# iclavera/learning_to_adapt

Measured on AMD Instinct MI355X. Metric: controller-steps/sec (n_cand=2000, H=30, ens=5), higher is better.
Workload: dtype f32

## Files before the change

learning_to_adapt_amd/csrc/l2a_api.hip:

```cpp

#define L2A_PACK_KERNELS 1
#include "l2a_host.h"
#include "l2a_kernels.h"
#include "l2a_valu.h"
#include "l2a_adapt.h"
#include "l2a_mfma_launch.h"
#include "l2a_micro_pack.h"
#include "l2a_micro_launch.h"

#include <chrono>
#include <cmath>
#include <cstdio>
#include <cstdlib>
#include <cstring>
#include <string>
#include <vector>

#include <immintrin.h>
#include <unistd.h>

namespace {

std::string g_init_error;

// ... 66 lines not shown
int allow_big_lds(const l2a_ctx* ctx, K kernel, int bytes) {
    L2A_HIP(ctx, hipFuncSetAttribute(reinterpret_cast<const void*>(kernel),
                                     hipFuncAttributeMaxDynamicSharedMemorySize, bytes));
    return L2A_OK;
}

int split_mode_for(const l2a_model* md, int e_loop) {
    const int policy = md->ctx->split_policy;
    if (policy == 0) return 0;
    if ((e_loop & 1) && md->n_hidden >= 2 && policy == 1) return 2;
    return (e_loop >= 2) ? 1 : 0;
}

int choose_nt(const l2a_model* md, int m, int n, int e_loop, int sa_bytes_nt2, int other_bytes_nt2) {
    const int cus = md->ctx->num_cu > 0 ? md->ctx->num_cu : 256;
    if (2 * sa_bytes_nt2 + other_bytes_nt2 > md->ctx->lds_per_block) return 1;
    if (md->TPW >= 8 || md->OT >= 4) return 1;
    static const int force_nt = [] { const char* e = std::getenv("L2A_FORCE_NT"); return (e && (e[0] == '1' || e[0] == '2')) ? e[0] - '0' : 0; }();
    if (force_nt) return force_nt;
    const long long wg1 = (long long)m * ceil_div(n, 16);
    const long long wg2 = (long long)m * ceil_div(n, 32);
    const long long t = wg1 % cus;
    double cost1 = (double)((wg1 + cus - 1) / cus);
    if (wg1 > cus && t != 0 && 2 * t <= cus && split_mode_for(md, e_loop) != 0) cost1 = (double)(wg1 / cus) + 0.8;
    const double cost2 = (double)((wg2 + cus - 1) / cus) * 1.9;
    return (cost2 < cost1) ? 2 : 1;
}

int sa_elems_for(const l2a_model* md, int nt) {
    const int ht = md->H / 16;
    const int a = nt * ht;
    const int b = L2A_NW * nt * md->OT;
    return (a > b ? a : b) * 64;
}

int launch_rollout(l2a_model* md, L2AKParams& p, void* stream_v) {
    l2a_ctx* ctx = md->ctx;
    l2a_device_guard guard(ctx->device);
    hipStream_t stream = reinterpret_cast<hipStream_t>(stream_v);
    const int sets_needed = ctx->dry ? 0 : (p.mode == L2A_MODE_PER_BLOCK) ? (p.m < md->n_sets ? p.m : md->n_sets) : md->n_sets;
    for (int e = 0; e < sets_needed; ++e) {
        if (!md->weights_set[e]) return fail(ctx, L2A_ESTATE, "weight set " + std::to_string(e) + " was never set");
        if (!md->norm_set[e]) return fail(ctx, L2A_ESTATE, "normalisation of set " + std::to_string(e) + " was never set");
    }
    if (p.mode == L2A_MODE_PER_BLOCK && p.m > md->n_sets)
        return fail(ctx, L2A_EINVAL, "per-block mode needs one weight set per env/block");
    p.c_lo = 0; p.c_hi = p.n; p.done_total = 0;

    int kind = ctx->kernel_kind;
    if (kind == L2A_KERNEL_AUTO) kind = md->mfma_ok ? L2A_KERNEL_MFMA : L2A_KERNEL_VALU;
    if (kind == L2A_KERNEL_MFMA && !md->mfma_ok)
        return fail(ctx, L2A_EINVAL, "model shape is not eligible for the MFMA kernel "
                                     "(needs equal hidden widths of 128/256/512, obs_dim<=64, act_dim<=16)");

    const int e_loop0 = (p.mode == L2A_MODE_MEAN) ? md->n_sets : 1;
    const int cus0 = ctx->num_cu > 0 ? ctx->num_cu : 256;
    const int cst_set = 32 * md->KG0 + 48 * md->OT + md->n_hidden * md->H;
    auto lds_plan = [&](int nt_, int nseq, int x_bytes, int* lb_out, int* cst_off_out) {
        const int sa = sa_elems_for(md, nt_);
        const int ps_bytes = L2A_NW * nt_ * md->OT * 64 * 16;
        const int cst_bytes_all = nseq * cst_set * 4;
        int lb_ = 1, part_bytes = 0;
        if (md->n_hidden == 2 && ctx->batch_sets != 1) {
            const int cap = ctx->batch_sets > 0 ? ctx->batch_sets : 4;
            for (int lb = (nseq < cap ? nseq : cap); lb >= 2; --lb) {
                const int pbytes = lb * ps_bytes;
                if (lb * sa * 16 + pbytes + cst_bytes_all + x_bytes <= ctx->lds_per_block) {
                    lb_ = lb;
                    part_bytes = pbytes;
                    break;
                }
            }
        }
        *lb_out = lb_;
        *cst_off_out = ((lb_ > 1 ? lb_ : 2) * sa * 16 + part_bytes) / 16;
        return *cst_off_out * 16 + cst_bytes_all + x_bytes;
    };
    int front_k = 0;
    if (kind == L2A_KERNEL_MFMA) {
        const long long tiles1 = (long long)p.m * ceil_div(p.n, 16);
        int lb2 = 1, off2 = 0;
        if (ctx->double_policy != 0 && md->TPW == 8 && md->OT <= 3 && tiles1 >= 2LL * cus0 &&
            lds_plan(2, e_loop0, 0, &lb2, &off2) <= ctx->lds_per_block) {
            const long long D = tiles1 / (2LL * cus0);
            const long long R = tiles1 - 2LL * cus0 * D;
            if (R == 0 || 2 * R > 3LL * cus0) front_k = ceil_div(p.n, 32);
            else front_k = (int)((cus0 * D) / p.m);
            if (32LL * front_k >= p.n) front_k = ceil_div(p.n, 32);
        }
    }
    const int n_front = (32LL * front_k >= p.n) ? (front_k ? p.n : 0) : 32 * front_k;
    const int n_rest = p.n - n_front;

    bool micro = false;
    int mc_W = 0, mc_hi = 0, mc_quads = 0, smem_m = 0;
    long long mc_span = 0;
    if (kind == L2A_KERNEL_MFMA && n_rest > 0 && md->micro_ok && ctx->micro_policy != 0) {
        const long long tiles16 = (long long)p.m * ceil_div(n_rest, 16);
        const int quads = ceil_div(n_rest, 4);
        int W = cus0 / p.m;
        if (W > quads) W = quads;
        const int hi = W > 0 ? ceil_div(quads, W) : 99;
        if (hi >= 1 && hi <= 3) W = ceil_div(quads, hi);
        const int smem_need = l2a_mlp_micro_smem(md->H, md->KG0, md->n_hidden, e_loop0);
        const long long span = (long long)((p.mode == L2A_MODE_PER_BLOCK ? p.m : e_loop0) - 1) * md->set_stride * 4 +
                               l2a_mlp_micro_floats(md->H, md->KG0, md->n_hidden) * 4;
// ... 161 lines not shown
        rc = L2A_OK;
        if (rc != L2A_OK) return rc;
    } else {
        p.tiles_per_env = ceil_div(p.n, L2A_VT);
        const int smem = (md->in_dim + 2 * md->hmax + 3 * md->obs_dim + md->act_dim + 1) * L2A_VT * 4;
        if (smem > ctx->lds_per_block)
            return fail(ctx, L2A_EINVAL, "LDS budget exceeded by the VALU kernel (" + std::to_string(smem) + " B)");
        if (ctx->dry) {
            const int g[12] = {0, 0, 0, -1, 0, p.m * p.tiles_per_env, smem, 1, 0, 0, 0, 0};
            std::memcpy(ctx->dry, g, sizeof(g));
            return L2A_OK;
        }
        int rc = allow_big_lds(ctx, l2a_rollout_valu_k, smem);
        if (rc != L2A_OK) return rc;
        const dim3 grid((unsigned)(p.m * p.tiles_per_env)), block(256);
        hipLaunchKernelGGL(l2a_rollout_valu_k, grid, block, smem, stream, p);
    }
    L2A_HIP(ctx, hipGetLastError());
    return L2A_OK;
}

void model_shape(l2a_model* md, int obs_dim, int act_dim, int n_hidden, const int* hidden, int hidden_act, int output_act,
                 int n_sets, int mode) {
    md->obs_dim = obs_dim; md->act_dim = act_dim; md->in_dim = obs_dim + act_dim;
    md->n_hidden = n_hidden;
    md->hmax = 0;
    for (int i = 0; i < n_hidden; ++i) {
        md->hidden[i] = hidden[i];
        if (hidden[i] > md->hmax) md->hmax = hidden[i];
    }
    md->hidden_act = hidden_act; md->output_act = output_act;
    md->n_sets = n_sets; md->mode = mode;
    md->KG0 = ceil_div(md->in_dim, 16);
    md->OT = ceil_div(obs_dim, 16);
    md->mfma_ok = mfma_eligible(obs_dim, act_dim, n_hidden, hidden);
    md->H = md->mfma_ok ? hidden[0] : 0;
    md->TPW = md->mfma_ok ? hidden[0] / (16 * L2A_NW) : 0;
    md->micro_ok = md->mfma_ok && (md->H == 256 || md->H == 512);
    md->m_o4 = (md->micro_ok && md->OT == 2 && md->KG0 == 2 && n_hidden > 1 && obs_dim - 16 <= 4) ? 1 : 0;
}

void fill_model_params(const l2a_model* md, L2AKParams& p) {
    std::memset(&p, 0, sizeof(p));
    p.wblk = md->wblk;
    p.set_stride = md->set_stride;
    for (int i = 0; i < L2A_MAX_LAYERS; ++i) {
        p.raw_w[i] = md->raw_w[i];
        p.raw_b[i] = md->raw_b[i];
        p.hidden[i] = md->hidden[i];
    }
    p.pk_w0 = md->pk_w0; p.pk_wmid = md->pk_wmid; p.pk_wmid_stride = md->pk_wmid_stride;
    p.pk_wout = md->pk_wout; p.pk_bout = md->pk_bout; p.nm_off = md->nm_off;
    p.pk_m = md->pk_m; p.m_o4 = md->m_o4;
    p.m_nrec = md->micro_ok ? l2a_mlp_micro_nrec(md->H, md->KG0, md->n_hidden) : 0;
    p.n_hidden = md->n_hidden;
    p.obs_dim = md->obs_dim; p.act_dim = md->act_dim; p.in_dim = md->in_dim;
    p.hidden_act = md->hidden_act; p.output_act = md->output_act;
    p.mode = md->mode; p.n_sets = md->n_sets;
    p.KG0 = md->KG0; p.OT = md->OT; p.hmax = md->hmax;
    p.hid_floor = (md->hidden_act == L2A_ACT_RELU) ? 0.0f : -INFINITY;
    p.out_floor = (md->output_act == L2A_ACT_RELU) ? 0.0f : -INFINITY;
}

}

extern "C" {

int l2a_init(int device, l2a_ctx** out) {
    if (!out) return fail(nullptr, L2A_EINVAL, "l2a_init: out is null");
    *out = nullptr;
    int count = 0;
    hipError_t e = hipGetDeviceCount(&count);
    if (e != hipSuccess || count <= 0)
        return fail(nullptr, L2A_ENODEV, std::string("no HIP device visible: ") +
                                             (e != hipSuccess ? hipGetErrorString(e) : "device count is 0"));
    if (device < 0 || device >= count)
        return fail(nullptr, L2A_EINVAL, "device index " + std::to_string(device) + " out of range");
    hipDeviceProp_t prop;
    e = hipGetDeviceProperties(&prop, device);
    if (e != hipSuccess) return fail(nullptr, L2A_EHIP, std::string("hipGetDeviceProperties: ") + hipGetErrorString(e));
    std::string arch(prop.gcnArchName);
    if (arch.rfind("gfx950", 0) != 0)
        return fail(nullptr, L2A_ENODEV, "libl2a_hip.so is built for gfx950 only; device reports " + arch);
    e = hipSetDevice(device);
    if (e != hipSuccess) return fail(nullptr, L2A_EHIP, std::string("hipSetDevice: ") + hipGetErrorString(e));
    l2a_ctx* ctx = new l2a_ctx();
    ctx->device = device;
    ctx->num_cu = prop.multiProcessorCount;
    ctx->lds_per_block = (int)prop.sharedMemPerBlock;
    if (ctx->lds_per_block < 160 * 1024) ctx->lds_per_block = 160 * 1024;
    ctx->clock_khz = prop.clockRate;
    ctx->arch = arch;
    ctx->name = prop.name;
    e = hipHostMalloc(reinterpret_cast<void**>(&ctx->status_host), sizeof(unsigned int), hipHostMallocMapped);
    if (e == hipSuccess) {
        *ctx->status_host = 0;
        e = hipHostGetDevicePointer(reinterpret_cast<void**>(&ctx->status_dev), ctx->status_host, 0);
    }
    if (e != hipSuccess) {
        std::string msg = std::string("allocating the launch status word: ") + hipGetErrorString(e);
        delete ctx;
        return fail(nullptr, L2A_EHIP, msg);
    }
    const char* sp = std::getenv("L2A_SPLIT");
    if (sp && sp[0] >= '0' && sp[0] <= '2') ctx->split_policy = sp[0] - '0';
    const char* xa = std::getenv("L2A_XCD_ALIGN");
// ... 820 lines not shown
```

learning_to_adapt_amd/csrc/l2a_kernels.h:

```cpp
#pragma once

#include <hip/hip_runtime.h>

#include "../../include/l2a.h"

#define L2A_MAX_LAYERS 9
#define L2A_OTMAX 4
#define L2A_KG0MAX 5

typedef float f32x4 __attribute__((ext_vector_type(4)));

#define L2A_SC1 16

struct L2AKParams {
    const float* wblk;
    long long set_stride;
    long long raw_w[L2A_MAX_LAYERS];
    long long raw_b[L2A_MAX_LAYERS];
    long long pk_w0;
    long long pk_wmid;
    long long pk_wmid_stride;
    long long pk_wout;
    long long pk_bout;
    long long nm_off;
    int hidden[L2A_MAX_LAYERS];
    int n_hidden;
    int obs_dim, act_dim, in_dim;
    int hidden_act, output_act;
    int mode, n_sets;
    int KG0, OT;
    int sa_elems;
    int cst_set;
    int lb;
    int cst_off;
    int n_cst;
    float hid_floor, out_floor;
    long long pk_m;
    int m_nrec, m_o4;
    long long m_bytes;
    int mc_w, mc_r, mc_hi;
    int hmax;
    const float* obs0;
    const float* actions;
    float* returns_out;
    unsigned long long* best_key;
    float* state_out;
    const float* ret_in;
    double disc0;
    int obs_per_row;
    int m, n, h;
    int tiles_per_env;
    int c_lo, c_hi;
    int done_total;
    int cand_offset;
    double discount;
    l2a_reward rw;
    int split;
    int pl_units, pl_f, pl_r, pl_w;
    int split_from;
    unsigned int xtag;
    unsigned long long* xbuf;
    unsigned int* status;
    unsigned int spin_limit;
    unsigned long long* dbg;
    unsigned int* done_ctr;
    unsigned long long* mail_keys;
    unsigned long long* mail_seq_ptr;
    unsigned long long mail_seq;
    unsigned long long* next_keys;
};

__host__ __device__ inline void l2a_pack_decode(long long idx, int KG, int* k, int* u) {
    const int ii = (int)(idx & 3);
    const int lane = (int)((idx >> 2) & 63);
    const long long rest = idx >> 8;
    const int g = (int)(rest % KG);
    const int c = (int)(rest / KG);
    *k = 16 * g + 4 * (lane >> 4) + ii;
    *u = 16 * c + (lane & 15);
}

__device__ __forceinline__ float l2a_max_nan(float x, float f) { return __builtin_elementwise_maximum(x, f); }

__device__ __forceinline__ float l2a_act1(float x, int kind) {
    switch (kind) {
        case L2A_ACT_RELU: return l2a_max_nan(x, 0.0f);
        case L2A_ACT_TANH: return tanhf(x);
        case L2A_ACT_SIGMOID: return 1.0f / (1.0f + expf(-x));
        case L2A_ACT_SWISH: return x / (1.0f + expf(-x));
// ... 56 lines not shown
```

learning_to_adapt_amd/csrc/l2a_mfma.h:

```cpp
#pragma once

#include <type_traits>

#include "l2a_kernels.h"

#ifndef L2A_XEARLY
#define L2A_XEARLY 1
#endif

#ifndef L2A_NW
#define L2A_NW 4
#endif

typedef unsigned int u32x4 __attribute__((ext_vector_type(4)));
__device__ __forceinline__ __amdgpu_buffer_rsrc_t l2a_rsrc(const void* base, long long bytes) {
    return __builtin_amdgcn_make_buffer_rsrc(const_cast<void*>(base), 0, (int)bytes, 0x00020000);
}
__device__ __forceinline__ f32x4 l2a_ldw(__amdgpu_buffer_rsrc_t rs, int voff, int soff) {
    return __builtin_bit_cast(f32x4, __builtin_amdgcn_raw_buffer_load_b128(rs, voff, soff, 0));
}

template <bool GACT>
__device__ __forceinline__ f32x4 l2a_actv(f32x4 v, int kind, float floor) {
    if (GACT) return l2a_act4(v, kind);
// ... 4 lines not shown

__device__ __forceinline__ float l2a_sum_xor16(float x) {
    const unsigned int u = __float_as_uint(x);
    const auto r = __builtin_amdgcn_permlane16_swap(u, u, false, false);
    return __uint_as_float(r[0]) + __uint_as_float(r[1]);
}
__device__ __forceinline__ float l2a_sum_xor32(float x) {
    const unsigned int u = __float_as_uint(x);
    const auto r = __builtin_amdgcn_permlane32_swap(u, u, false, false);
    return __uint_as_float(r[0]) + __uint_as_float(r[1]);
}

#define L2A_MFMA4(a, b, c) __builtin_amdgcn_mfma_f32_4x4x1f32((a), (b), (c), 0, 0, 0)

#define L2A_OPAQUE(v) asm volatile("" : "+v"(v))

#ifndef L2A_TIMELINE
#define L2A_TS(slot)
#else
#define L2A_TS(slot)                                                                        \
    if (p.dbg && pairid == 0 && e < 8 && grp < 2) {                                         \
        unsigned long long ts_;                                                             \
        asm volatile("s_memtime %0\n\ts_waitcnt lgkmcnt(0)" : "=s"(ts_) : : "memory");       \
        if (lane == 0) p.dbg[(((long long)(grp * p.h + t) * 8 + e) * 8 + wave) * 16 + (slot)] = ts_; \
    }
#endif

#define L2A_STAGE_MFMA(CA, CB)                                                             \
    _Pragma("unroll") for (int ii = 0; ii < 4; ++ii)                                       \
        _Pragma("unroll") for (int nt = 0; nt < NT; ++nt)                                  \
            _Pragma("unroll") for (int tt = TW - 1; tt >= 0; --tt)    \
                acc[nt][tt] = L2A_MFMA(CA[tt][ii], CB[nt][ii], acc[nt][tt]);

#define L2A_STAGE(CA, CB, FA, FB, SOFF, IMM, GF)                                           \
    {                                                                                      \
        _Pragma("unroll") for (int tt = 0; tt < TW; ++tt)                                  \
            FA[tt] = l2a_ldw(rs, voff[tt] + (IMM), (SOFF));                                \
        _Pragma("unroll") for (int nt = 0; nt < NT; ++nt)                                  \
            FB[nt] = hin[(nt * HT + (GF)) * 64 + lane];                                    \
        L2A_STAGE_MFMA(CA, CB)                                                             \
         \
        __builtin_amdgcn_sched_group_barrier(0x100, NT, 0);                                \
        _Pragma("unroll") for (int tt = 0; tt < TW; ++tt) {                                \
            __builtin_amdgcn_sched_group_barrier(0x008, 4 * NT, 0);                        \
            __builtin_amdgcn_sched_group_barrier(0x020, 1, 0);                             \
        }                                                                                  \
        __builtin_amdgcn_sched_barrier(0);                                                 \
    }

#define L2A_PFT_MAX 6
#define L2A_PFT(TW_, OT_) ((OT_) <= 2 ? ((TW_) < L2A_PFT_MAX ? (TW_) : L2A_PFT_MAX) : ((TW_) < 2 ? (TW_) : 2))

template <int NT, int TW, int TPW, int OT, bool LAST>
__device__ __forceinline__ void l2a_hidden_gemm(__amdgpu_buffer_rsrc_t rs, __amdgpu_buffer_rsrc_t rsn,
                                                const int (&voff)[TPW], const int (&voffn)[TPW], int twn,
                                                int tile0, const f32x4* hin,
                                                f32x4 (&aA)[TPW], f32x4 (&aB)[TPW],
                                                f32x4 (&pfO)[TPW][OT], f32x4 (&acc)[NT][TPW], int lane,
                                                const float* bias_lds, f32x4 (&bias)[TPW], const int (&olane)[OT]) {
    constexpr int HT = L2A_NW * TPW;
    static_assert(HT % 4 == 0, "the k-group pipeline is unrolled by 4");
    f32x4 aC[TW], aD[TW], bA[NT], bB[NT], bC[NT], bD[NT];
#pragma unroll
    for (int nt = 0; nt < NT; ++nt) {
        bA[nt] = hin[(nt * HT + 0) * 64 + lane];
        bB[nt] = hin[(nt * HT + 1) * 64 + lane];
#pragma unroll
        for (int tt = 0; tt < TW; ++tt) acc[nt][tt] = (f32x4){0.f, 0.f, 0.f, 0.f};
    }
#pragma unroll
    for (int nt = 0; nt < NT; ++nt) { L2A_OPAQUE(bA[nt]); L2A_OPAQUE(bB[nt]); }
    __builtin_amdgcn_sched_barrier(0);

#pragma unroll 1
    for (int g = 0; g < HT - 4; g += 4) {
        const int soff = (g + 2) * 1024;
        L2A_STAGE(aA, bA, aC, bC, soff, 0, g + 2)
        L2A_STAGE(aB, bB, aD, bD, soff, 1024, g + 3)
        L2A_STAGE(aC, bC, aA, bA, soff, 2048, g + 4)
        L2A_STAGE(aD, bD, aB, bB, soff, 3072, g + 5)
    }
    L2A_STAGE(aA, bA, aC, bC, (HT - 2) * 1024, 0, HT - 2)
    L2A_STAGE(aB, bB, aD, bD, (HT - 2) * 1024, 1024, HT - 1)
    {
        if (LAST) {
#pragma unroll
            for (int tt = 0; tt < L2A_PFT(TW, OT); ++tt)
#pragma unroll
                for (int c = 0; c < OT; ++c)
                    if (((tt * OT + c) & 1) == 0)
                        pfO[tt][c] = l2a_ldw(rsn, olane[c] + (tile0 + tt) * 1024, c * HT * 1024);
        } else {
#pragma unroll
            for (int tt = 0; tt < TPW; ++tt)
                if (tt < twn) aA[tt] = l2a_ldw(rsn, voffn[tt], 0);
        }
        L2A_STAGE_MFMA(aC, bC)
        __builtin_amdgcn_sched_barrier(0);
    }
    {
#pragma unroll
        for (int tt = 0; tt < TW; ++tt) bias[tt] = *reinterpret_cast<const f32x4*>(bias_lds + 16 * tt);
        if (LAST) {
#pragma unroll
            for (int tt = 0; tt < L2A_PFT(TW, OT); ++tt)
#pragma unroll
                for (int c = 0; c < OT; ++c)
                    if (((tt * OT + c) & 1) == 1)
                        pfO[tt][c] = l2a_ldw(rsn, olane[c] + (tile0 + tt) * 1024, c * HT * 1024);
        } else {
#pragma unroll
            for (int tt = 0; tt < TPW; ++tt)
                if (tt < twn) aB[tt] = l2a_ldw(rsn, voffn[tt] + 1024, 0);
        }
        L2A_STAGE_MFMA(aD, bD)
        __builtin_amdgcn_sched_barrier(0);
    }
}

template <int NT, int TW, int TPW, int OT, int NPF, bool O4, class PF>
__device__ __forceinline__ void l2a_out_phase(const f32x4 (&hreg)[NT][TPW], f32x4 (&pfO)[TPW][OT],
                                              __amdgpu_buffer_rsrc_t rs_out, int tile0, PF prefetch,
                                              f32x4* pbuf, int chunk0, int lane, const int (&olane)[OT]) {
    constexpr int HT = L2A_NW * TPW;
    constexpr int CS = TPW / 2;
    constexpr int NCH = TW / CS;
    f32x4 a[TW][OT];
#pragma unroll
    for (int tt = 0; tt < TW; ++tt)
#pragma unroll
        for (int c = 0; c < OT; ++c)
            a[tt][c] = (tt < L2A_PFT(TW, OT)) ? pfO[tt][c]
                                              : l2a_ldw(rs_out, olane[c] + (tile0 + tt) * 1024, c * HT * 1024);
    prefetch();
    f32x4 acc[NCH][NT][OT];
#pragma unroll
    for (int ch = 0; ch < NCH; ++ch)
#pragma unroll
        for (int nt = 0; nt < NT; ++nt)
#pragma unroll
            for (int c = 0; c < OT; ++c) acc[ch][nt][c] = (f32x4){0.f, 0.f, 0.f, 0.f};
#pragma unroll
    for (int t2 = 0; t2 < CS; ++t2)
#pragma unroll
        for (int ii = 0; ii < 4; ++ii)
#pragma unroll
            for (int ch = 0; ch < NCH; ++ch)
#pragma unroll
                for (int nt = 0; nt < NT; ++nt)
#pragma unroll
                    for (int c = 0; c < OT; ++c)
                        acc[ch][nt][c] = (O4 && c == OT - 1)
                            ? L2A_MFMA4(a[ch * CS + t2][c][ii], hreg[nt][ch * CS + t2][ii], acc[ch][nt][c])
                            : L2A_MFMA(a[ch * CS + t2][c][ii], hreg[nt][ch * CS + t2][ii], acc[ch][nt][c]);
    {
        constexpr int NLATE = (TW - L2A_PFT(TW, OT)) * OT;
        constexpr int NMFMA = TW * 4 * NT * OT;
#pragma unroll
        for (int i = 0; i < NLATE; ++i) {
            __builtin_amdgcn_sched_group_barrier(0x020, 1, 0);
            __builtin_amdgcn_sched_group_barrier(0x008, 2, 0);
        }
        constexpr int PER = (NMFMA - 2 * NLATE) / NPF > 0 ? (NMFMA - 2 * NLATE) / NPF : 1;
#pragma unroll
        for (int i = 0; i < NPF; ++i) {
            __builtin_amdgcn_sched_group_barrier(0x008, PER, 0);
            __builtin_amdgcn_sched_group_barrier(0x020, 1, 0);
        }
    }
#pragma unroll
    for (int nt = 0; nt < NT; ++nt)
#pragma unroll
        for (int c = 0; c < OT; ++c)
            pbuf[((chunk0 * NT + nt) * OT + c) * 64 + lane] = (NCH == 2) ? acc[0][nt][c] + acc[NCH - 1][nt][c] : acc[0][nt][c];
}

template <int NT, int TPW, int OT, int KG0, bool GACT, int K0L = 4, bool N1 = false, bool O4 = false, bool FAN = false, bool WHOLE = false>
__global__ void __launch_bounds__(64 * L2A_NW) l2a_rollout_mfma_k(const L2AKParams p) {
    static_assert(!(FAN && WHOLE), "an instance is general, member fan or whole-tiles-only");
    constexpr bool NOHALF = FAN || WHOLE;
    constexpr int HT = L2A_NW * TPW;
    constexpr int TH = TPW / 2;
    static_assert(TPW % 2 == 0, "half members split a wave's tiles in two");
    constexpr int CST_BOUT = 32 * KG0 + 32 * OT;
    constexpr int CST_BHID = CST_BOUT + 16 * OT;
    constexpr int PS = L2A_NW * NT * OT * 64;
// ... 132 lines not shown
        for (int nt = 0; nt < NT; ++nt)
#pragma unroll
            for (int s = 0; s < 2; ++s)
#pragma unroll
                for (int ii = 0; ii < 4; ++ii)
                    dst[nt][s][ii] = __builtin_bit_cast(float, __builtin_amdgcn_raw_buffer_load_b32(ars, aoff[nt][s][ii], 0, 0));
    };
    f32x4 av[NT][2];
    float asq[NT];
    auto take_actions = [&](int t_fetch) {
#pragma unroll
        for (int nt = 0; nt < NT; ++nt) {
            av[nt][0] = av_next[nt][0];
            av[nt][1] = av_next[nt][1];
            float s = 0.0f;
#pragma unroll
            for (int ii = 0; ii < 4; ++ii) {
                s = fmaf(av[nt][0][ii], av[nt][0][ii], s);
                s = fmaf(av[nt][1][ii], av[nt][1][ii], s);
            }
            asq[nt] = s;
        }
        load_actions((t_fetch < p.h) ? t_fetch : p.h - 1, av_next);
    };
    load_actions(0, av_next);
    take_actions(1);

    float ret[NT];
#pragma unroll
    for (int nt = 0; nt < NT; ++nt) ret[nt] = p.ret_in ? p.ret_in[(long long)env * p.n + (valid[nt] ? cand[nt] : p.c_hi - 1)] : 0.0f;

    f32x4* hcur = buf0;
    f32x4* hoth = buf1;
    const float e_count = (float)e_loop;
    const float e_inv = 1.0f / e_count;
    double disc_pow = p.disc0;
    unsigned int spin_left = p.spin_limit;
    const unsigned int xtag0 = p.xtag;
    const __amdgpu_buffer_rsrc_t xrs = l2a_rsrc(p.xbuf, FAN ? (long long)n_pairs * e_loop * 2 * (NT * OT * 2 * 64 * 16)
                                                        : split ? (long long)n_pairs * 8 * (NT * OT * 2 * 64 * 16) : 16);

    constexpr int KG0P = (FAN && KG0 <= 2) ? KG0 : 1;
    f32x4 pfL0[KG0P][TPW];
    f32x4 pfA[TPW], pfB[TPW];
    f32x4 pfO[TPW][OT];
    int voff[TPW], voffh[TPW], voff0[TPW];
    const int tile0h = grp * (HT / 2) + wave * TH;
#pragma unroll
    for (int tt = 0; tt < TPW; ++tt) {
        voff[tt] = lane * 16 + (c0 + tt) * HT * 1024;
        voffh[tt] = lane * 16 + (tile0h + (tt < TH ? tt : 0)) * HT * 1024;
        voff0[tt] = lane * 16 + (c0 + tt) * KG0 * 1024;
    }
    const long long w0_bytes = (long long)HT * KG0 * 1024, wm_bytes = (long long)HT * HT * 1024,
                    wo_bytes = (long long)OT * HT * 1024;
    {
        const __amdgpu_buffer_rsrc_t r0 = l2a_rsrc(set_base(seq(0)) + p.pk_w0, w0_bytes);
#pragma unroll
        for (int g = 0; g < KG0P; ++g)
#pragma unroll
            for (int tt = 0; tt < TPW; ++tt) pfL0[g][tt] = l2a_ldw(r0, voff0[tt] + g * 1024, 0);
    }

    for (int t = 0; t < p.h; ++t) {
        f32x4 dsum[NT][OT], dgrp[NT][OT], qsh[NT][OT];
#pragma unroll
        for (int nt = 0; nt < NT; ++nt)
#pragma unroll
            for (int c = 0; c < OT; ++c) {
                dsum[nt][c] = (f32x4){0.f, 0.f, 0.f, 0.f};
                dgrp[nt][c] = (f32x4){0.f, 0.f, 0.f, 0.f};
                qsh[nt][c] = (f32x4){0.f, 0.f, 0.f, 0.f};
            }

        const unsigned int xtag = xtag0 + (unsigned int)(t + 1);
        constexpr int XREG = NT * OT * 2 * 64 * 16;
        auto xbase = [&](int g, int region) { return (((lpair * 2 + g) * 2 + (t & 1)) * 2 + region) * XREG + lane * 16; };
        auto xput = [&](int region, const f32x4 (&v)[NT][OT]) {
#pragma unroll
            for (int nt = 0; nt < NT; ++nt)
#pragma unroll
                for (int c = 0; c < OT; ++c)
#pragma unroll
                    for (int hh = 0; hh < 2; ++hh) {
                        u32x4 g;
                        g.x = xtag; g.y = __float_as_uint(v[nt][c][2 * hh]);
                        g.z = xtag; g.w = __float_as_uint(v[nt][c][2 * hh + 1]);
                        __builtin_amdgcn_raw_buffer_store_b128(g, xrs, xbase(grp, region) + ((nt * OT + c) * 2 + hh) * 1024, 0, L2A_SC1);
                    }
        };
        auto xget = [&](int region, f32x4 (&v)[NT][OT]) {
            bool ok = true;
#pragma unroll
            for (int nt = 0; nt < NT; ++nt)
#pragma unroll
                for (int c = 0; c < OT; ++c)
#pragma unroll
                    for (int hh = 0; hh < 2; ++hh) {
                        const u32x4 g = __builtin_amdgcn_raw_buffer_load_b128(
                            xrs, xbase(grp ^ 1, region) + ((nt * OT + c) * 2 + hh) * 1024, 0, L2A_SC1);
                        v[nt][c][2 * hh] = __uint_as_float(g.y);
                        v[nt][c][2 * hh + 1] = __uint_as_float(g.w);
                        ok = ok && (g.x == xtag) && (g.z == xtag);
                    }
            return ok;
        };

        bool xearly = false;
        u32x4 sw[2][NT][OT][2];
        for (int b0 = 0; b0 < n_seq; b0 += LB) {
            const int nb = (n_seq - b0 < LB) ? n_seq - b0 : LB;
            f32x4 hreg[NT][TPW];

            auto layer0 = [&](int j, auto last_tag) {
                constexpr bool last_l0 = decltype(last_tag)::value;
                const int i = b0 + j;
                const int e = seq(i);
                const float* wb = set_base(e);
                const float* nr = nrm + i * NRM_SET;
                const __amdgpu_buffer_rsrc_t rs_out = l2a_rsrc(wb + p.pk_wout, wo_bytes);
                L2A_TS(0)
                const __amdgpu_buffer_rsrc_t r0 = l2a_rsrc(wb + p.pk_w0, w0_bytes);
                f32x4 a[KG0][TPW];
#pragma unroll
                for (int g = 0; g < KG0; ++g)
#pragma unroll
                    for (int tt = 0; tt < TPW; ++tt)
                        a[g][tt] = (g < KG0P) ? pfL0[g < KG0P ? g : 0][tt] : l2a_ldw(r0, voff0[tt] + g * 1024, 0);
                L2A_TS(8)
                constexpr bool XPRE = (KG0 <= 2);
                auto norm_in = [&](int g, const f32x4& mu, const f32x4& iv, f32x4 (&x)[NT]) {
#pragma unroll
                    for (int nt = 0; nt < NT; ++nt) {
                        f32x4 sv = (f32x4){0.f, 0.f, 0.f, 0.f};
                        if (g < OT) sv = st[nt][g < OT ? g : 0];
                        f32x4 aa = (f32x4){0.f, 0.f, 0.f, 0.f};
                        if (g == ga0) aa = av[nt][0];
                        if (g == ga0 + 1) aa = av[nt][1];
#pragma unroll
                        for (int ii = 0; ii < 4; ++ii) x[nt][ii] = ((sv[ii] + aa[ii]) - mu[ii]) * iv[ii];
                    }
                };
                f32x4 xin[XPRE ? KG0 : 1][NT];
                if (XPRE) {
                    f32x4 mu[KG0], iv[KG0];
#pragma unroll
                    for (int g = 0; g < KG0; ++g) {
                        mu[g] = *reinterpret_cast<const f32x4*>(nr + 16 * g + 4 * qq);
                        iv[g] = *reinterpret_cast<const f32x4*>(nr + 16 * KG0 + 16 * g + 4 * qq);
                    }
                    __builtin_amdgcn_sched_barrier(0);
#pragma unroll
                    for (int g = 0; g < KG0; ++g) norm_in(g, mu[g], iv[g], xin[XPRE ? g : 0]);
                }
                f32x4 bias0[TPW];
#pragma unroll
                for (int tt = 0; tt < TPW; ++tt)
                    bias0[tt] = *reinterpret_cast<const f32x4*>(nr + CST_BHID + 16 * (c0 + tt) + 4 * qq);
                f32x4 acc[NT][TPW];
                auto l0_mfma = [&](auto npf_tag) {
                    constexpr int NPF = decltype(npf_tag)::value;
#pragma unroll
                    for (int nt = 0; nt < NT; ++nt)
#pragma unroll
                        for (int tt = 0; tt < TPW; ++tt) acc[nt][tt] = (f32x4){0.f, 0.f, 0.f, 0.f};
#pragma unroll
                    for (int g = 0; g < KG0; ++g) {
                        f32x4 xg[NT];
                        if (XPRE) {
#pragma unroll
                            for (int nt = 0; nt < NT; ++nt) xg[nt] = xin[XPRE ? g : 0][nt];
                        } else {
                            const f32x4 mu = *reinterpret_cast<const f32x4*>(nr + 16 * g + 4 * qq);
                            const f32x4 iv = *reinterpret_cast<const f32x4*>(nr + 16 * KG0 + 16 * g + 4 * qq);
                            norm_in(g, mu, iv, xg);
                        }
#pragma unroll
                        for (int ii = 0; ii < 4; ++ii) {
                            if (g == KG0 - 1 && ii >= K0L) continue;
#pragma unroll
                            for (int nt = 0; nt < NT; ++nt)
#pragma unroll
                                for (int tt = 0; tt < TPW; ++tt)
                                    acc[nt][tt] = L2A_MFMA(a[g][tt][ii], xg[nt][ii], acc[nt][tt]);
                        }
                    }
                    constexpr int NM = ((KG0 - 1) * 4 + K0L) * NT * TPW;
                    constexpr int PER = NM / (NPF > 0 ? NPF : 1) > 0 ? NM / (NPF > 0 ? NPF : 1) : 1;
                    __builtin_amdgcn_sched_group_barrier(0x020, (KG0 - KG0P) * TPW, 0);
#pragma unroll
                    for (int k = 0; k < NPF; ++k) {
                        __builtin_amdgcn_sched_group_barrier(0x008, PER, 0);
                        __builtin_amdgcn_sched_group_barrier(0x020, 1, 0);
                    }
                };
                if (N1) {
#pragma unroll
                    for (int tt = 0; tt < L2A_PFT(TPW, OT); ++tt)
#pragma unroll
                        for (int c = 0; c < OT; ++c)
                            pfO[tt][c] = l2a_ldw(rs_out, olane[c] + (c0 + tt) * 1024, c * HT * 1024);
                    l0_mfma(std::integral_constant<int, L2A_PFT(TPW, OT) * OT>{});
                } else if (!last_l0) {
                    const __amdgpu_buffer_rsrc_t r0n = l2a_rsrc(set_base(seq(i + 1)) + p.pk_w0, w0_bytes);
#pragma unroll
                    for (int g = 0; g < KG0P; ++g)
#pragma unroll
                        for (int tt = 0; tt < TPW; ++tt) pfL0[g][tt] = l2a_ldw(r0n, voff0[tt] + g * 1024, 0);
                    l0_mfma(std::integral_constant<int, KG0P * TPW>{});
                } else {
                    const int e0 = seq(b0);
                    const __amdgpu_buffer_rsrc_t rs1 = l2a_rsrc(set_base(e0) + p.pk_wmid, wm_bytes);
                    const bool next_half = !NOHALF && (e0 == e_shared) && n_hidden == 2;
                    if (next_half) {
#pragma unroll
                        for (int tt = 0; tt < TH; ++tt) {
                            pfA[tt] = l2a_ldw(rs1, voffh[tt], 0);
                            pfB[tt] = l2a_ldw(rs1, voffh[tt] + 1024, 0);
                        }
                        l0_mfma(std::integral_constant<int, 2 * TH>{});
                    } else {
#pragma unroll
                        for (int tt = 0; tt < TPW; ++tt) {
                            pfA[tt] = l2a_ldw(rs1, voff[tt], 0);
                            pfB[tt] = l2a_ldw(rs1, voff[tt] + 1024, 0);
                        }
                        l0_mfma(std::integral_constant<int, 2 * TPW>{});
                    }
                }
                L2A_TS(9)
#pragma unroll
                for (int tt = 0; tt < TPW; ++tt) {
#pragma unroll
                    for (int nt = 0; nt < NT; ++nt)
                        hreg[nt][tt] = l2a_actv<GACT>(acc[nt][tt] + bias0[tt], p.hidden_act, p.hid_floor);
                }
                L2A_TS(10)
                if (!N1) {
                    f32x4* hdst = (LB > 1) ? buf0 + j * p.sa_elems : hcur;
#pragma unroll
                    for (int tt = 0; tt < TPW; ++tt)
#pragma unroll
                        for (int nt = 0; nt < NT; ++nt) hdst[(nt * HT + c0 + tt) * 64 + lane] = hreg[nt][tt];
                }
                L2A_TS(1)
            };

            auto member = [&](int j, auto last_tag) {
                constexpr bool last_set = decltype(last_tag)::value;
                const int i = b0 + j;
                const int e = seq(i);
                const bool is_half = !NOHALF && last_set && (e == e_shared);
                const float* wb = set_base(e);
                const float* nr = nrm + i * NRM_SET;
                const __amdgpu_buffer_rsrc_t rs_out = l2a_rsrc(wb + p.pk_wout, wo_bytes);
                f32x4* pb = (LB > 1) ? pbase + j * PS : hoth;
                L2A_TS(2)
                if (!N1) {
                    f32x4 acc[NT][TPW], bias[TPW];
                    for (int l = 1; last_set && l < n_hidden - 1; ++l) {
                        const float* wl = wb + p.pk_wmid + (long long)(l - 1) * p.pk_wmid_stride;
                        const bool next_half = is_half && (l == n_hidden - 2);
                        l2a_hidden_gemm<NT, TPW, TPW, OT, false>(l2a_rsrc(wl, wm_bytes), l2a_rsrc(wl + p.pk_wmid_stride, wm_bytes),
                                                                 voff, next_half ? voffh : voff, next_half ? TH : TPW, 0,
                                                                 hcur, pfA, pfB, pfO, acc, lane,
                                                                 nr + CST_BHID + l * (16 * HT) + 16 * c0 + 4 * qq, bias, olane);
#pragma unroll
                        for (int tt = 0; tt < TPW; ++tt) {
#pragma unroll
                            for (int nt = 0; nt < NT; ++nt)
                                hoth[(nt * HT + c0 + tt) * 64 + lane] = l2a_actv<GACT>(acc[nt][tt] + bias[tt], p.hidden_act, p.hid_floor);
                        }
                        __syncthreads();
                        f32x4* tmp = hcur; hcur = hoth; hoth = tmp;
                    }
                    if (LB == 1) pb = hoth;
                    L2A_TS(15)
                    const f32x4* hin = (LB > 1) ? buf0 + j * p.sa_elems : hcur;
                    const __amdgpu_buffer_rsrc_t rs_last =
                        l2a_rsrc(wb + p.pk_wmid + (long long)(n_hidden - 2) * p.pk_wmid_stride, wm_bytes);
                    const float* bl = nr + CST_BHID + (n_hidden - 1) * (16 * HT);
                    if (!is_half) {
                        l2a_hidden_gemm<NT, TPW, TPW, OT, true>(rs_last, rs_out, voff, voff, TPW, c0, hin, pfA, pfB, pfO,
                                                                acc, lane, bl + 16 * c0 + 4 * qq, bias, olane);
#pragma unroll
                        for (int tt = 0; tt < TPW; ++tt) {
#pragma unroll
                            for (int nt = 0; nt < NT; ++nt)
                                hreg[nt][tt] = l2a_actv<GACT>(acc[nt][tt] + bias[tt], p.hidden_act, p.hid_floor);
                        }
                    } else {
                        l2a_hidden_gemm<NT, TH, TPW, OT, true>(rs_last, rs_out, voffh, voffh, TH, tile0h, hin, pfA, pfB,
                                                               pfO, acc, lane, bl + 16 * tile0h + 4 * qq, bias, olane);
#pragma unroll
                        for (int tt = 0; tt < TH; ++tt) {
#pragma unroll
                            for (int nt = 0; nt < NT; ++nt)
                                hreg[nt][tt] = l2a_actv<GACT>(acc[nt][tt] + bias[tt], p.hidden_act, p.hid_floor);
                        }
                    }
                }
                L2A_TS(3)
                if (last_set) {
                    const __amdgpu_buffer_rsrc_t r0n = l2a_rsrc(set_base(seq((i + 1 < n_seq) ? i + 1 : 0)) + p.pk_w0, w0_bytes);
                    auto pf_l0 = [&]() {
#pragma unroll
                        for (int g = 0; g < KG0P; ++g)
#pragma unroll
                            for (int tt = 0; tt < TPW; ++tt) pfL0[g][tt] = l2a_ldw(r0n, voff0[tt] + g * 1024, 0);
                    };
                    if (is_half) l2a_out_phase<NT, TH, TPW, OT, KG0P * TPW, O4>(hreg, pfO, rs_out, tile0h, pf_l0, pb, wave, lane, olane);
                    else l2a_out_phase<NT, TPW, TPW, OT, KG0P * TPW, O4>(hreg, pfO, rs_out, c0, pf_l0, pb, wave, lane, olane);
                } else {
                    const int en = seq(i + 1);
                    const __amdgpu_buffer_rsrc_t rsn = l2a_rsrc(set_base(en) + p.pk_wmid, wm_bytes);
                    if (!NOHALF && en == e_shared) {
                        l2a_out_phase<NT, TPW, TPW, OT, 2 * TH, O4>(hreg, pfO, rs_out, c0, [&]() {
#pragma unroll
                            for (int tt = 0; tt < TH; ++tt) {
                                pfA[tt] = l2a_ldw(rsn, voffh[tt], 0);
                                pfB[tt] = l2a_ldw(rsn, voffh[tt] + 1024, 0);
                            }
                        }, pb, wave, lane, olane);
                    } else {
                        l2a_out_phase<NT, TPW, TPW, OT, 2 * TPW, O4>(hreg, pfO, rs_out, c0, [&]() {
#pragma unroll
                            for (int tt = 0; tt < TPW; ++tt) {
                                pfA[tt] = l2a_ldw(rsn, voff[tt], 0);
                                pfB[tt] = l2a_ldw(rsn, voff[tt] + 1024, 0);
                            }
                        }, pb, wave, lane, olane);
                    }
                }
                L2A_TS(4)
            };
            for (int j = 0; j + 1 < nb; ++j) layer0(j, std::false_type{});
            layer0(nb - 1, std::true_type{});
            if (!N1) __syncthreads();
            for (int j = 0; j + 1 < nb; ++j) member(j, std::false_type{});
            member(nb - 1, std::true_type{});

            __syncthreads();
            constexpr bool XE_OK = L2A_XEARLY && !NOHALF && NT == 1 && OT <= 2 && KG0 <= 2;
            const bool xe = XE_OK && split == 2 && nb >= 2 && b0 + nb == n_seq;
            for (int jj = 0; jj < nb; ++jj) {
                const int j = (xe && wave == 0) ? (jj == 0 ? nb - 1 : jj - 1) : jj;
                const int i = b0 + j;
                const int e = seq(i);
                const bool is_half = !NOHALF && (e == e_shared);
                const float* nr = nrm + i * NRM_SET;
                const f32x4* pb = (LB > 1) ? pbase + j * PS : hoth;
                L2A_TS(5)
                if (e == e_half && !split) {
#pragma unroll
                    for (int nt = 0; nt < NT; ++nt)
#pragma unroll
                        for (int c = 0; c < OT; ++c) {
                            dsum[nt][c] = dgrp[nt][c];
                            dgrp[nt][c] = (f32x4){0.f, 0.f, 0.f, 0.f};
                        }
                }
#pragma unroll
                for (int c = 0; c < OT; ++c) {
                    f32x4 part[L2A_NW][NT];
#pragma unroll
                    for (int ch = 0; ch < L2A_NW; ++ch)
#pragma unroll
                        for (int nt = 0; nt < NT; ++nt) part[ch][nt] = pb[((ch * NT + nt) * OT + c) * 64 + lane];
                    const f32x4 bias = *reinterpret_cast<const f32x4*>(nr + CST_BOUT + 16 * c + 4 * qq);
                    const f32x4 omu = *reinterpret_cast<const f32x4*>(nr + 32 * KG0 + 16 * c + 4 * qq);
                    const f32x4 osd = *reinterpret_cast<const f32x4*>(nr + 32 * KG0 + 16 * OT + 16 * c + 4 * qq);
                    __builtin_amdgcn_sched_barrier(0);
#pragma unroll
                    for (int nt = 0; nt < NT; ++nt) {
                        static_assert(L2A_NW == 4, "the canonical tree below is written out for four waves");
                        f32x4 s = (part[0][nt] + part[1][nt]) + (part[2][nt] + part[3][nt]);
                        if (is_half) {
                            qsh[nt][c] = s;
                        } else {
                            if (O4 && c == OT - 1) {
#pragma unroll
                                for (int ii = 0; ii < 4; ++ii) s[ii] = l2a_sum_xor32(l2a_sum_xor16(s[ii]));
// ... 338 lines not shown
```

Baseline: 702.6.

## Use one weight-block buffer resource with scalar offsets and peel first hidden-GEMM stage

Replaces the per-set, per-layer buffer resource descriptors with a single descriptor covering the whole weight block, addressing each set and layer through int scalar offsets. This removes repeated 128-bit descriptor construction and the SGPR pressure that comes with it. It also peels the first stage of the hidden GEMM when NT==1, so the accumulator is seeded by the first MFMA instead of being zeroed, and adds sched_group_barrier hints to interleave the loads. Models whose weights exceed 2 GiB are now rejected from the MFMA path.

```diff
diff --git a/learning_to_adapt_amd/csrc/l2a_api.hip b/learning_to_adapt_amd/csrc/l2a_api.hip
--- a/learning_to_adapt_amd/csrc/l2a_api.hip
+++ b/learning_to_adapt_amd/csrc/l2a_api.hip
@@ -142,6 +142,8 @@
     if (kind == L2A_KERNEL_MFMA && !md->mfma_ok)
         return fail(ctx, L2A_EINVAL, "model shape is not eligible for the MFMA kernel "
                                      "(needs equal hidden widths of 128/256/512, obs_dim<=64, act_dim<=16)");
+    if (kind == L2A_KERNEL_MFMA && md->set_stride * md->n_sets * 4 >= (1LL << 31))
+        return fail(ctx, L2A_EINVAL, "the model's weight block exceeds 2 GiB: not eligible for the MFMA kernel (use the VALU kernel)");
 
     const int e_loop0 = (p.mode == L2A_MODE_MEAN) ? md->n_sets : 1;
     const int cus0 = ctx->num_cu > 0 ? ctx->num_cu : 256;
@@ -409,6 +411,12 @@
     p.pk_w0 = md->pk_w0; p.pk_wmid = md->pk_wmid; p.pk_wmid_stride = md->pk_wmid_stride;
     p.pk_wout = md->pk_wout; p.pk_bout = md->pk_bout; p.nm_off = md->nm_off;
     p.pk_m = md->pk_m; p.m_o4 = md->m_o4;
+    if (md->mfma_ok && md->set_stride * md->n_sets * 4 < (1LL << 31)) {
+        p.wb_total = (int)(md->set_stride * md->n_sets * 4);
+        p.wb_set = (int)(md->set_stride * 4);
+        p.wb_w0 = (int)(md->pk_w0 * 4); p.wb_wmid = (int)(md->pk_wmid * 4);
+        p.wb_wmid_stride = (int)(md->pk_wmid_stride * 4); p.wb_wout = (int)(md->pk_wout * 4);
+    }
     p.m_nrec = md->micro_ok ? l2a_mlp_micro_nrec(md->H, md->KG0, md->n_hidden) : 0;
     p.n_hidden = md->n_hidden;
     p.obs_dim = md->obs_dim; p.act_dim = md->act_dim; p.in_dim = md->in_dim;
diff --git a/learning_to_adapt_amd/csrc/l2a_kernels.h b/learning_to_adapt_amd/csrc/l2a_kernels.h
--- a/learning_to_adapt_amd/csrc/l2a_kernels.h
+++ b/learning_to_adapt_amd/csrc/l2a_kernels.h
@@ -35,6 +35,7 @@
     int cst_off;
     int n_cst;
     float hid_floor, out_floor;
+    int wb_total, wb_set, wb_w0, wb_wmid, wb_wmid_stride, wb_wout;
     long long pk_m;
     int m_nrec, m_o4;
     long long m_bytes;
diff --git a/learning_to_adapt_amd/csrc/l2a_mfma.h b/learning_to_adapt_amd/csrc/l2a_mfma.h
--- a/learning_to_adapt_amd/csrc/l2a_mfma.h
+++ b/learning_to_adapt_amd/csrc/l2a_mfma.h
@@ -80,7 +80,7 @@
 #define L2A_PFT(TW_, OT_) ((OT_) <= 2 ? ((TW_) < L2A_PFT_MAX ? (TW_) : L2A_PFT_MAX) : ((TW_) < 2 ? (TW_) : 2))
 
 template <int NT, int TW, int TPW, int OT, bool LAST>
-__device__ __forceinline__ void l2a_hidden_gemm(__amdgpu_buffer_rsrc_t rs, __amdgpu_buffer_rsrc_t rsn,
+__device__ __forceinline__ void l2a_hidden_gemm(__amdgpu_buffer_rsrc_t rs, int sb, int sbn,
                                                 const int (&voff)[TPW], const int (&voffn)[TPW], int twn,
                                                 int tile0, const f32x4* hin,
                                                 f32x4 (&aA)[TPW], f32x4 (&aB)[TPW],
@@ -93,23 +93,57 @@
     for (int nt = 0; nt < NT; ++nt) {
         bA[nt] = hin[(nt * HT + 0) * 64 + lane];
         bB[nt] = hin[(nt * HT + 1) * 64 + lane];
-#pragma unroll
-        for (int tt = 0; tt < TW; ++tt) acc[nt][tt] = (f32x4){0.f, 0.f, 0.f, 0.f};
-    }
-#pragma unroll
-    for (int nt = 0; nt < NT; ++nt) { L2A_OPAQUE(bA[nt]); L2A_OPAQUE(bB[nt]); }
-    __builtin_amdgcn_sched_barrier(0);
-
+    }
+    constexpr bool PEEL = (NT == 1);
+    if constexpr (PEEL) {
+#pragma unroll
+        for (int tt = 0; tt < TW; ++tt) aC[tt] = l2a_ldw(rs, voff[tt], sb + 2 * 1024);
+#pragma unroll
+        for (int nt = 0; nt < NT; ++nt) bC[nt] = hin[(nt * HT + 2) * 64 + lane];
+#pragma unroll
+        for (int ii = 0; ii < 4; ++ii)
+#pragma unroll
+            for (int nt = 0; nt < NT; ++nt)
+#pragma unroll
+                for (int tt = TW - 1; tt >= 0; --tt)
+                    acc[nt][tt] = L2A_MFMA(aA[tt][ii], bA[nt][ii], (ii == 0 ? (f32x4){0.f, 0.f, 0.f, 0.f} : acc[nt][tt]));
+        __builtin_amdgcn_sched_group_barrier(0x100, NT, 0);
+#pragma unroll
+        for (int tt = 0; tt < TW; ++tt) {
+            __builtin_amdgcn_sched_group_barrier(0x008, 4 * NT, 0);
+            __builtin_amdgcn_sched_group_barrier(0x020, 1, 0);
+        }
+        __builtin_amdgcn_sched_barrier(0);
+#pragma unroll
+        for (int nt = 0; nt < NT; ++nt) { L2A_OPAQUE(bB[nt]); L2A_OPAQUE(bC[nt]); }
+        __builtin_amdgcn_sched_barrier(0);
 #pragma unroll 1
-    for (int g = 0; g < HT - 4; g += 4) {
-        const int soff = (g + 2) * 1024;
-        L2A_STAGE(aA, bA, aC, bC, soff, 0, g + 2)
-        L2A_STAGE(aB, bB, aD, bD, soff, 1024, g + 3)
-        L2A_STAGE(aC, bC, aA, bA, soff, 2048, g + 4)
-        L2A_STAGE(aD, bD, aB, bB, soff, 3072, g + 5)
-    }
-    L2A_STAGE(aA, bA, aC, bC, (HT - 2) * 1024, 0, HT - 2)
-    L2A_STAGE(aB, bB, aD, bD, (HT - 2) * 1024, 1024, HT - 1)
+        for (int g = 1; g < HT - 3; g += 4) {
+            const int soff = sb + (g + 2) * 1024;
+            L2A_STAGE(aB, bB, aD, bD, soff, 0, g + 2)
+            L2A_STAGE(aC, bC, aA, bA, soff, 1024, g + 3)
+            L2A_STAGE(aD, bD, aB, bB, soff, 2048, g + 4)
+            L2A_STAGE(aA, bA, aC, bC, soff, 3072, g + 5)
+        }
+    } else {
+#pragma unroll
+        for (int nt = 0; nt < NT; ++nt)
+#pragma unroll
+            for (int tt = 0; tt < TW; ++tt) acc[nt][tt] = (f32x4){0.f, 0.f, 0.f, 0.f};
+#pragma unroll
+        for (int nt = 0; nt < NT; ++nt) { L2A_OPAQUE(bA[nt]); L2A_OPAQUE(bB[nt]); }
+        __builtin_amdgcn_sched_barrier(0);
+#pragma unroll 1
+        for (int g = 0; g < HT - 4; g += 4) {
+            const int soff = sb + (g + 2) * 1024;
+            L2A_STAGE(aA, bA, aC, bC, soff, 0, g + 2)
+            L2A_STAGE(aB, bB, aD, bD, soff, 1024, g + 3)
+            L2A_STAGE(aC, bC, aA, bA, soff, 2048, g + 4)
+            L2A_STAGE(aD, bD, aB, bB, soff, 3072, g + 5)
+        }
+        L2A_STAGE(aA, bA, aC, bC, sb + (HT - 2) * 1024, 0, HT - 2)
+    }
+    L2A_STAGE(aB, bB, aD, bD, sb + (HT - 2) * 1024, 1024, HT - 1)
     {
         if (LAST) {
 #pragma unroll
@@ -117,11 +151,11 @@
 #pragma unroll
                 for (int c = 0; c < OT; ++c)
                     if (((tt * OT + c) & 1) == 0)
-                        pfO[tt][c] = l2a_ldw(rsn, olane[c] + (tile0 + tt) * 1024, c * HT * 1024);
+                        pfO[tt][c] = l2a_ldw(rs, olane[c] + (tile0 + tt) * 1024, sbn + c * HT * 1024);
         } else {
 #pragma unroll
             for (int tt = 0; tt < TPW; ++tt)
-                if (tt < twn) aA[tt] = l2a_ldw(rsn, voffn[tt], 0);
+                if (tt < twn) aA[tt] = l2a_ldw(rs, voffn[tt], sbn);
         }
         L2A_STAGE_MFMA(aC, bC)
         __builtin_amdgcn_sched_barrier(0);
@@ -135,11 +169,11 @@
 #pragma unroll
                 for (int c = 0; c < OT; ++c)
                     if (((tt * OT + c) & 1) == 1)
-                        pfO[tt][c] = l2a_ldw(rsn, olane[c] + (tile0 + tt) * 1024, c * HT * 1024);
+                        pfO[tt][c] = l2a_ldw(rs, olane[c] + (tile0 + tt) * 1024, sbn + c * HT * 1024);
         } else {
 #pragma unroll
             for (int tt = 0; tt < TPW; ++tt)
-                if (tt < twn) aB[tt] = l2a_ldw(rsn, voffn[tt] + 1024, 0);
+                if (tt < twn) aB[tt] = l2a_ldw(rs, voffn[tt] + 1024, sbn);
         }
         L2A_STAGE_MFMA(aD, bD)
         __builtin_amdgcn_sched_barrier(0);
@@ -148,7 +182,7 @@
 
 template <int NT, int TW, int TPW, int OT, int NPF, bool O4, class PF>
 __device__ __forceinline__ void l2a_out_phase(const f32x4 (&hreg)[NT][TPW], f32x4 (&pfO)[TPW][OT],
-                                              __amdgpu_buffer_rsrc_t rs_out, int tile0, PF prefetch,
+                                              __amdgpu_buffer_rsrc_t rs_out, int so_out, int tile0, PF prefetch,
                                               f32x4* pbuf, int chunk0, int lane, const int (&olane)[OT]) {
     constexpr int HT = L2A_NW * TPW;
     constexpr int CS = TPW / 2;
@@ -159,7 +193,7 @@
 #pragma unroll
         for (int c = 0; c < OT; ++c)
             a[tt][c] = (tt < L2A_PFT(TW, OT)) ? pfO[tt][c]
-                                              : l2a_ldw(rs_out, olane[c] + (tile0 + tt) * 1024, c * HT * 1024);
+                                              : l2a_ldw(rs_out, olane[c] + (tile0 + tt) * 1024, so_out + c * HT * 1024);
     prefetch();
     f32x4 acc[NCH][NT][OT];
 #pragma unroll
@@ -398,15 +432,13 @@
         voffh[tt] = lane * 16 + (tile0h + (tt < TH ? tt : 0)) * HT * 1024;
         voff0[tt] = lane * 16 + (c0 + tt) * KG0 * 1024;
     }
-    const long long w0_bytes = (long long)HT * KG0 * 1024, wm_bytes = (long long)HT * HT * 1024,
-                    wo_bytes = (long long)OT * HT * 1024;
-    {
-        const __amdgpu_buffer_rsrc_t r0 = l2a_rsrc(set_base(seq(0)) + p.pk_w0, w0_bytes);
-#pragma unroll
-        for (int g = 0; g < KG0P; ++g)
-#pragma unroll
-            for (int tt = 0; tt < TPW; ++tt) pfL0[g][tt] = l2a_ldw(r0, voff0[tt] + g * 1024, 0);
-    }
+    const __amdgpu_buffer_rsrc_t rW = l2a_rsrc(p.wblk, p.wb_total);
+    const int wb_set = p.wb_set;
+    auto set_off = [&](int i) { return (per_block ? env : seq(i)) * wb_set; };
+#pragma unroll
+    for (int g = 0; g < KG0P; ++g)
+#pragma unroll
+        for (int tt = 0; tt < TPW; ++tt) pfL0[g][tt] = l2a_ldw(rW, voff0[tt] + g * 1024, set_off(0) + p.wb_w0);
 
     for (int t = 0; t < p.h; ++t) {
         f32x4 dsum[NT][OT], dgrp[NT][OT], qsh[NT][OT];
@@ -462,17 +494,15 @@
                 constexpr bool last_l0 = decltype(last_tag)::value;
                 const int i = b0 + j;
                 const int e = seq(i);
-                const float* wb = set_base(e);
+                const int so = set_off(i);
                 const float* nr = nrm + i * NRM_SET;
-                const __amdgpu_buffer_rsrc_t rs_out = l2a_rsrc(wb + p.pk_wout, wo_bytes);
                 L2A_TS(0)
-                const __amdgpu_buffer_rsrc_t r0 = l2a_rsrc(wb + p.pk_w0, w0_bytes);
                 f32x4 a[KG0][TPW];
 #pragma unroll
                 for (int g = 0; g < KG0; ++g)
 #pragma unroll
                     for (int tt = 0; tt < TPW; ++tt)
-                        a[g][tt] = (g < KG0P) ? pfL0[g < KG0P ? g : 0][tt] : l2a_ldw(r0, voff0[tt] + g * 1024, 0);
+                        a[g][tt] = (g < KG0P) ? pfL0[g < KG0P ? g : 0][tt] : l2a_ldw(rW, voff0[tt] + g * 1024, so + p.wb_w0);
                 L2A_TS(8)
                 constexpr bool XPRE = (KG0 <= 2);
                 auto norm_in = [&](int g, const f32x4& mu, const f32x4& iv, f32x4 (&x)[NT]) {
@@ -545,31 +575,31 @@
                     for (int tt = 0; tt < L2A_PFT(TPW, OT); ++tt)
 #pragma unroll
                         for (int c = 0; c < OT; ++c)
-                            pfO[tt][c] = l2a_ldw(rs_out, olane[c] + (c0 + tt) * 1024, c * HT * 1024);
+                            pfO[tt][c] = l2a_ldw(rW, olane[c] + (c0 + tt) * 1024, so + p.wb_wout + c * HT * 1024);
                     l0_mfma(std::integral_constant<int, L2A_PFT(TPW, OT) * OT>{});
                 } else if (!last_l0) {
-                    const __amdgpu_buffer_rsrc_t r0n = l2a_rsrc(set_base(seq(i + 1)) + p.pk_w0, w0_bytes);
+                    const int son = set_off(i + 1) + p.wb_w0;
 #pragma unroll
                     for (int g = 0; g < KG0P; ++g)
 #pragma unroll
-                        for (int tt = 0; tt < TPW; ++tt) pfL0[g][tt] = l2a_ldw(r0n, voff0[tt] + g * 1024, 0);
+                        for (int tt = 0; tt < TPW; ++tt) pfL0[g][tt] = l2a_ldw(rW, voff0[tt] + g * 1024, son);
                     l0_mfma(std::integral_constant<int, KG0P * TPW>{});
                 } else {
                     const int e0 = seq(b0);
-                    const __amdgpu_buffer_rsrc_t rs1 = l2a_rsrc(set_base(e0) + p.pk_wmid, wm_bytes);
+                    const int so1 = set_off(b0) + p.wb_wmid;
                     const bool next_half = !NOHALF && (e0 == e_shared) && n_hidden == 2;
                     if (next_half) {
 #pragma unroll
                         for (int tt = 0; tt < TH; ++tt) {
-                            pfA[tt] = l2a_ldw(rs1, voffh[tt], 0);
-                            pfB[tt] = l2a_ldw(rs1, voffh[tt] + 1024, 0);
+                            pfA[tt] = l2a_ldw(rW, voffh[tt], so1);
+                            pfB[tt] = l2a_ldw(rW, voffh[tt] + 1024, so1);
                         }
                         l0_mfma(std::integral_constant<int, 2 * TH>{});
                     } else {
 #pragma unroll
                         for (int tt = 0; tt < TPW; ++tt) {
-                            pfA[tt] = l2a_ldw(rs1, voff[tt], 0);
-                            pfB[tt] = l2a_ldw(rs1, voff[tt] + 1024, 0);
+                            pfA[tt] = l2a_ldw(rW, voff[tt], so1);
+                            pfB[tt] = l2a_ldw(rW, voff[tt] + 1024, so1);
                         }
                         l0_mfma(std::integral_constant<int, 2 * TPW>{});
                     }
@@ -597,17 +627,17 @@
                 const int i = b0 + j;
                 const int e = seq(i);
                 const bool is_half = !NOHALF && last_set && (e == e_shared);
-                const float* wb = set_base(e);
+                const int so = set_off(i);
+                const int so_out = so + p.wb_wout;
                 const float* nr = nrm + i * NRM_SET;
-                const __amdgpu_buffer_rsrc_t rs_out = l2a_rsrc(wb + p.pk_wout, wo_bytes);
                 f32x4* pb = (LB > 1) ? pbase + j * PS : hoth;
                 L2A_TS(2)
                 if (!N1) {
                     f32x4 acc[NT][TPW], bias[TPW];
                     for (int l = 1; last_set && l < n_hidden - 1; ++l) {
-                        const float* wl = wb + p.pk_wmid + (long long)(l - 1) * p.pk_wmid_stride;
+                        const int sl = so + p.wb_wmid + (l - 1) * p.wb_wmid_stride;
                         const bool next_half = is_half && (l == n_hidden - 2);
-                        l2a_hidden_gemm<NT, TPW, TPW, OT, false>(l2a_rsrc(wl, wm_bytes), l2a_rsrc(wl + p.pk_wmid_stride, wm_bytes),
+                        l2a_hidden_gemm<NT, TPW, TPW, OT, false>(rW, sl, sl + p.wb_wmid_stride,
                                                                  voff, next_half ? voffh : voff, next_half ? TH : TPW, 0,
                                                                  hcur, pfA, pfB, pfO, acc, lane,
                                                                  nr + CST_BHID + l * (16 * HT) + 16 * c0 + 4 * qq, bias, olane);
@@ -623,11 +653,10 @@
                     if (LB == 1) pb = hoth;
                     L2A_TS(15)
                     const f32x4* hin = (LB > 1) ? buf0 + j * p.sa_elems : hcur;
-                    const __amdgpu_buffer_rsrc_t rs_last =
-                        l2a_rsrc(wb + p.pk_wmid + (long long)(n_hidden - 2) * p.pk_wmid_stride, wm_bytes);
+                    const int so_last = so + p.wb_wmid + (n_hidden - 2) * p.wb_wmid_stride;
                     const float* bl = nr + CST_BHID + (n_hidden - 1) * (16 * HT);
                     if (!is_half) {
-                        l2a_hidden_gemm<NT, TPW, TPW, OT, true>(rs_last, rs_out, voff, voff, TPW, c0, hin, pfA, pfB, pfO,
+                        l2a_hidden_gemm<NT, TPW, TPW, OT, true>(rW, so_last, so_out, voff, voff, TPW, c0, hin, pfA, pfB, pfO,
                                                                 acc, lane, bl + 16 * c0 + 4 * qq, bias, olane);
 #pragma unroll
                         for (int tt = 0; tt < TPW; ++tt) {
@@ -636,7 +665,7 @@
                                 hreg[nt][tt] = l2a_actv<GACT>(acc[nt][tt] + bias[tt], p.hidden_act, p.hid_floor);
                         }
                     } else {
-                        l2a_hidden_gemm<NT, TH, TPW, OT, true>(rs_last, rs_out, voffh, voffh, TH, tile0h, hin, pfA, pfB,
+                        l2a_hidden_gemm<NT, TH, TPW, OT, true>(rW, so_last, so_out, voffh, voffh, TH, tile0h, hin, pfA, pfB,
                                                                pfO, acc, lane, bl + 16 * tile0h + 4 * qq, bias, olane);
 #pragma unroll
                         for (int tt = 0; tt < TH; ++tt) {
@@ -648,32 +677,32 @@
                 }
                 L2A_TS(3)
                 if (last_set) {
-                    const __amdgpu_buffer_rsrc_t r0n = l2a_rsrc(set_base(seq((i + 1 < n_seq) ? i + 1 : 0)) + p.pk_w0, w0_bytes);
+                    const int son = set_off((i + 1 < n_seq) ? i + 1 : 0) + p.wb_w0;
                     auto pf_l0 = [&]() {
 #pragma unroll
                         for (int g = 0; g < KG0P; ++g)
 #pragma unroll
-                            for (int tt = 0; tt < TPW; ++tt) pfL0[g][tt] = l2a_ldw(r0n, voff0[tt] + g * 1024, 0);
+                            for (int tt = 0; tt < TPW; ++tt) pfL0[g][tt] = l2a_ldw(rW, voff0[tt] + g * 1024, son);
                     };
-                    if (is_half) l2a_out_phase<NT, TH, TPW, OT, KG0P * TPW, O4>(hreg, pfO, rs_out, tile0h, pf_l0, pb, wave, lane, olane);
-                    else l2a_out_phase<NT, TPW, TPW, OT, KG0P * TPW, O4>(hreg, pfO, rs_out, c0, pf_l0, pb, wave, lane, olane);
+                    if (is_half) l2a_out_phase<NT, TH, TPW, OT, KG0P * TPW, O4>(hreg, pfO, rW, so_out, tile0h, pf_l0, pb, wave, lane, olane);
+                    else l2a_out_phase<NT, TPW, TPW, OT, KG0P * TPW, O4>(hreg, pfO, rW, so_out, c0, pf_l0, pb, wave, lane, olane);
                 } else {
                     const int en = seq(i + 1);
-                    const __amdgpu_buffer_rsrc_t rsn = l2a_rsrc(set_base(en) + p.pk_wmid, wm_bytes);
+                    const int sn = set_off(i + 1) + p.wb_wmid;
                     if (!NOHALF && en == e_shared) {
-                        l2a_out_phase<NT, TPW, TPW, OT, 2 * TH, O4>(hreg, pfO, rs_out, c0, [&]() {
+                        l2a_out_phase<NT, TPW, TPW, OT, 2 * TH, O4>(hreg, pfO, rW, so_out, c0, [&]() {
 #pragma unroll
                             for (int tt = 0; tt < TH; ++tt) {
-                                pfA[tt] = l2a_ldw(rsn, voffh[tt], 0);
-                                pfB[tt] = l2a_ldw(rsn, voffh[tt] + 1024, 0);
+                                pfA[tt] = l2a_ldw(rW, voffh[tt], sn);
+                                pfB[tt] = l2a_ldw(rW, voffh[tt] + 1024, sn);
                             }
                         }, pb, wave, lane, olane);
                     } else {
-                        l2a_out_phase<NT, TPW, TPW, OT, 2 * TPW, O4>(hreg, pfO, rs_out, c0, [&]() {
+                        l2a_out_phase<NT, TPW, TPW, OT, 2 * TPW, O4>(hreg, pfO, rW, so_out, c0, [&]() {
 #pragma unroll
                             for (int tt = 0; tt < TPW; ++tt) {
-                                pfA[tt] = l2a_ldw(rsn, voff[tt], 0);
-                                pfB[tt] = l2a_ldw(rsn, voff[tt] + 1024, 0);
+                                pfA[tt] = l2a_ldw(rW, voff[tt], sn);
+                                pfB[tt] = l2a_ldw(rW, voff[tt] + 1024, sn);
                             }
                         }, pb, wave, lane, olane);
                     }
```

New measurement: 700.3. About the same (-0.3%).
